# yanqinJiang/Animate3D

Measured on AMD Instinct MI355X. Metric: UNet denoise-steps/sec, 4view×16frame×512² MV-VDM @1/2/4/8 GPU, higher is better.
Workload: dtype bf16; 1 GPU; BASELINE config 2: 4 views x 16 frames x 512^2 px (64x64 latent), CFG-doubled batch V=8 videos, one MVUNetMotionModel.forward per step, SD1.5 MV-VDM UNet 1.53 B params, seeded synthetic weights; parallelism=single GPU

## Files before the change

animate3d_amd/csrc/temporal_attn.hip:

```cpp
#include "common.h"


namespace {

constexpr int SLAB = 320;
constexpr int SL = 40;
constexpr int NSL = SLAB / SL;

struct TAParams {
  const uint16_t* Q; const uint16_t* K; const uint16_t* V; int64_t ld;
  int64_t ldq;
  uint16_t* O; int64_t ldo;
  int videos, frames; int64_t L; int heads; float scale_log2;
  int64_t npix;
  int q_f0, q_frames, kv_fpr; int64_t kv_rs;
};

typedef short s16x4_t __attribute__((ext_vector_type(4)));
typedef _Float16 f16x4_t __attribute__((ext_vector_type(4)));
A3D_DEV f32x4_t mfma16k16(const u32x2_t& a, const u32x2_t& b, const f32x4_t& c) {
#ifdef A3D_STORAGE_F16
  return __builtin_amdgcn_mfma_f32_16x16x16f16(__builtin_bit_cast(f16x4_t, a), __builtin_bit_cast(f16x4_t, b), c, 0, 0, 0);
#else
  return __builtin_amdgcn_mfma_f32_16x16x16bf16_1k(__builtin_bit_cast(s16x4_t, a), __builtin_bit_cast(s16x4_t, b), c, 0, 0, 0);
#endif
}

template <int FP, int D>
__global__ __launch_bounds__(NSL * FP) void temporal_attn_mfma_kernel(const TAParams p) {
  constexpr int ROWB = SLAB + 8;
  constexpr int FB = FP / 16;
  constexpr int KS = (D + 15) / 16;
  constexpr int NH = SLAB / D;
  constexpr int NT = NSL * FP, NW = NT / 64;
  extern __shared__ __attribute__((aligned(16))) uint16_t smem[];
  const int F = p.frames;
  const int tid = threadIdx.x, lane = tid & 63, wid = tid >> 6;
  const int64_t pix = blockIdx.x < p.npix ? (int64_t)blockIdx.x : p.npix - 1;
  const int c0 = blockIdx.y * SLAB;
  const int64_t v = pix / p.L, l = pix % p.L;
  constexpr int chunks = SLAB / 8;

  auto src_of = [&](int it) -> const uint16_t* {
    const int ch = it % chunks;
    const int f = (it / chunks) % F;
    const int ten = it / (chunks * F);
    if (ten == 0) {
      int fq = f - p.q_f0;
      if (fq < 0 || fq >= p.q_frames) fq = 0;
      return p.Q + ((v * p.q_frames + fq) * p.L + l) * p.ldq + c0 + ch * 8;
    }
    const int64_t row = (int64_t)(f / p.kv_fpr) * p.kv_rs + (v * p.kv_fpr + f % p.kv_fpr) * p.L + l;
    return (ten == 1 ? p.K : p.V) + row * p.ld + c0 + ch * 8;
  };
  auto dst_of = [&](int it) -> uint16_t* {
// ... 1 lines not shown
    const int f = (it / chunks) % F;
    const int ten = it / (chunks * F);
    return smem + ((size_t)ten * F + f) * ROWB + ch * 8;
  };
  const int items = 3 * F * chunks;
  if (F == FP) {
    constexpr int ITEMS = 3 * FP * chunks, NIT = (ITEMS + NT - 1) / NT;
    u32x4_t stg[NIT];
#pragma unroll
    for (int k = 0; k < NIT; ++k) {
      const int it = tid + k * NT;
      if (ITEMS % NT == 0 || it < ITEMS) stg[k] = *reinterpret_cast<const u32x4_t*>(src_of(it));
    }
#pragma unroll
    for (int k = 0; k < NIT; ++k) {
      const int it = tid + k * NT;
      if (ITEMS % NT == 0 || it < ITEMS) *reinterpret_cast<u32x4_t*>(dst_of(it)) = stg[k];
    }
  } else {
    for (int it = tid; it < items; it += NT) *reinterpret_cast<u32x4_t*>(dst_of(it)) = *reinterpret_cast<const u32x4_t*>(src_of(it));
  }
  __syncthreads();

  const int i16 = lane & 15, k4 = lane >> 4;
  uint16_t* const Qs = smem;
  const uint16_t* const Ks = smem + (size_t)F * ROWB;
  const uint16_t* const Vs = smem + (size_t)2 * F * ROWB;
  for (int h = wid; h < NH; h += NW) {
    const int hc = h * D;
    f32x4_t sT[FB][FB];
    u32x2_t qfr[FB][KS];
#pragma unroll
    for (int ib = 0; ib < FB; ++ib) {
      const int fi = 16 * ib + i16 < F ? 16 * ib + i16 : F - 1;
#pragma unroll
      for (int ks = 0; ks < KS; ++ks) {
        u32x2_t w = *reinterpret_cast<const u32x2_t*>(Qs + (size_t)fi * ROWB + hc + 16 * ks + 4 * k4);
        if (16 * ks + 4 * k4 >= D) w = u32x2_t{0u, 0u};
        qfr[ib][ks] = w;
      }
    }
#pragma unroll
    for (int jb = 0; jb < FB; ++jb) {
      const int fj = 16 * jb + i16 < F ? 16 * jb + i16 : F - 1;
      u32x2_t kfr[KS];
#pragma unroll
      for (int ks = 0; ks < KS; ++ks) {
        kfr[ks] = *reinterpret_cast<const u32x2_t*>(Ks + (size_t)fj * ROWB + hc + 16 * ks + 4 * k4);
        if (16 * ks + 4 * k4 >= D) kfr[ks] = u32x2_t{0u, 0u};
      }
#pragma unroll
      for (int ib = 0; ib < FB; ++ib) {
        f32x4_t acc = {0.f, 0.f, 0.f, 0.f};
#pragma unroll
        for (int ks = 0; ks < KS; ++ks) acc = mfma16k16(kfr[ks], qfr[ib][ks], acc);
        sT[jb][ib] = acc;
      }
    }
    u32x2_t pfr[FB][FB];
    float inv[FB];
#pragma unroll
    for (int ib = 0; ib < FB; ++ib) {
      float mx = -INFINITY;
#pragma unroll
      for (int jb = 0; jb < FB; ++jb)
#pragma unroll
        for (int r = 0; r < 4; ++r) {
          const bool ok = 16 * jb + 4 * k4 + r < F;
          sT[jb][ib][r] = ok ? sT[jb][ib][r] * p.scale_log2 : -INFINITY;
          mx = fmaxf(mx, sT[jb][ib][r]);
        }
      mx = fmaxf(mx, __shfl_xor(mx, 16));
      mx = fmaxf(mx, __shfl_xor(mx, 32));
      float sum = 0.f;
#pragma unroll
      for (int jb = 0; jb < FB; ++jb) {
        float e[4];
#pragma unroll
        for (int r = 0; r < 4; ++r) { e[r] = __builtin_amdgcn_exp2f(sT[jb][ib][r] - mx); sum += e[r]; }
        pfr[jb][ib] = u32x2_t{pack16(e[0], e[1]), pack16(e[2], e[3])};
      }
      sum += __shfl_xor(sum, 16);
      sum += __shfl_xor(sum, 32);
      inv[ib] = 1.f / sum;
    }
#pragma unroll
    for (int db = 0; db < KS; ++db) {
      u32x2_t vfr[FB];
#pragma unroll
      for (int jb = 0; jb < FB; ++jb) {
        const int fj = 16 * jb + 4 * k4 + (i16 >> 2) < F ? 16 * jb + 4 * k4 + (i16 >> 2) : F - 1;
        vfr[jb] = lds_tr16_b64(Vs + (size_t)fj * ROWB + hc + 16 * db + 4 * (i16 & 3));
      }
#pragma unroll
      for (int ib = 0; ib < FB; ++ib) {
        f32x4_t o = {0.f, 0.f, 0.f, 0.f};
#pragma unroll
        for (int jb = 0; jb < FB; ++jb) o = mfma16k16(vfr[jb], pfr[jb][ib], o);
        const int fi = 16 * ib + i16;
        if (16 * db + 4 * k4 < D && fi < F) {
          const u32x2_t w = {pack16(o[0] * inv[ib], o[1] * inv[ib]), pack16(o[2] * inv[ib], o[3] * inv[ib])};
          *reinterpret_cast<u32x2_t*>(Qs + (size_t)fi * ROWB + hc + 16 * db + 4 * k4) = w;
        }
      }
    }
  }
  __syncthreads();
  if ((int64_t)blockIdx.x < p.npix) {
    for (int it = tid; it < p.q_frames * chunks; it += NT) {
      const int ch = it % chunks, fq = it / chunks;
      const u32x4_t w = *reinterpret_cast<const u32x4_t*>(Qs + (size_t)(p.q_f0 + fq) * ROWB + ch * 8);
      *reinterpret_cast<u32x4_t*>(p.O + ((v * p.q_frames + fq) * p.L + l) * p.ldo + c0 + ch * 8) = w;
    }
  }
}

template <int FP, int D>
int launch_mfma(hipStream_t s, const TAParams& p, int C) {
  if (p.npix > 0x7fffffffLL) return A3D_EINVAL;
  const size_t lds = (size_t)3 * p.frames * (SLAB + 8) * sizeof(uint16_t);
  static uint64_t attr_done = 0;
  if (int rc = a3d_once_per_device(attr_done, [] {
        return (int)hipFuncSetAttribute(reinterpret_cast<const void*>(&temporal_attn_mfma_kernel<FP, D>),
                                        hipFuncAttributeMaxDynamicSharedMemorySize, 3 * FP * (SLAB + 8) * 2); })) return rc;
  temporal_attn_mfma_kernel<FP, D><<<dim3((unsigned)p.npix, (unsigned)(C / SLAB)), dim3(NSL * FP), lds, s>>>(p);
  return a3d_launch_status();
}

template <int DP>
// ... 46 lines not shown
```

animate3d_amd/hip_ops.py:

```python
from __future__ import annotations

import ctypes
import os
from dataclasses import dataclass
from typing import Optional

import torch

_LIB_PATH = os.path.join(os.path.dirname(os.path.abspath(__file__)), "lib", "libanimate3d_hip.so")
_lib = None

c_i64, c_int, c_f32, c_vp = ctypes.c_int64, ctypes.c_int, ctypes.c_float, ctypes.c_void_p


class _RowMapC(ctypes.Structure):
    _fields_ = [("gdiv", c_i64), ("ga", c_i64), ("gb", c_i64), ("seg_len", c_i64), ("seg_stride", c_i64), ("ld", c_i64)]


@dataclass(frozen=True)
class RowMap:
    gdiv: int
    ga: int
    gb: int
    seg_len: int
# ... 15 lines not shown
    idx = rowmap_rows(m, groups, step, length, device)
    return bool(int(idx.min()) >= 0 and int(idx.max()) < rows and torch.unique(idx).numel() == rows)


_SIGNATURES = {
    "a3d_version": (ctypes.c_char_p, []),
    "a3d_gemm_bf16": (c_int, [c_vp, c_vp, c_i64, c_vp, c_i64, c_vp, c_vp, c_i64, c_vp, c_i64, c_vp, c_i64, c_i64, c_i64, c_i64, c_f32, c_f32, c_int]),
    "a3d_gemm_ws_bf16": (c_int, [c_vp, c_vp, c_i64, c_vp, c_i64, c_vp, c_vp, c_i64, c_vp, c_i64, c_vp, c_i64, c_i64, c_i64, c_i64, c_f32, c_f32, c_int,
                                 c_vp, c_i64, ctypes.POINTER(c_i64)]),
    "a3d_gemm2_bf16": (c_int, [c_vp, c_vp, c_i64, c_vp, c_i64, c_i64, c_vp, c_i64, c_vp, c_vp, c_i64, c_i64, c_i64, c_i64, c_int]),
    "a3d_gemm_geglu_bf16": (c_int, [c_vp, c_vp, c_i64, c_vp, c_i64, c_vp, c_vp, c_i64, c_i64, c_i64, c_i64, c_int]),
    "a3d_conv3x3_bf16": (c_int, [c_vp, c_vp, c_vp, c_vp, c_vp, c_i64, c_vp, c_vp, c_int, c_int, c_int, c_int, c_int, c_int, c_int, c_int]),
    "a3d_conv3x3_ws_bf16": (c_int, [c_vp, c_vp, c_vp, c_vp, c_vp, c_i64, c_vp, c_vp, c_int, c_int, c_int, c_int, c_int, c_int, c_int, c_int,
                                    c_vp, c_i64, ctypes.POINTER(c_i64)]),
    "a3d_flash_attn_bf16": (c_int, [c_vp, c_vp, c_vp, c_vp, c_vp, ctypes.POINTER(_RowMapC), ctypes.POINTER(_RowMapC), ctypes.POINTER(_RowMapC),
                                    c_int, c_int, c_int, c_i64, c_i64, c_f32, c_f32, c_int]),
    "a3d_flash_attn_counted_bf16": (c_int, [c_vp, c_vp, c_vp, c_vp, c_vp, ctypes.POINTER(_RowMapC), ctypes.POINTER(_RowMapC), ctypes.POINTER(_RowMapC),
                                            c_int, c_int, c_int, c_i64, c_i64, c_f32, c_f32, c_int, c_vp]),
    "a3d_flash_attn2_bf16": (c_int, [c_vp, c_vp, c_vp, c_vp, c_vp, c_vp, c_vp, ctypes.POINTER(_RowMapC), ctypes.POINTER(_RowMapC), ctypes.POINTER(_RowMapC),
                                     ctypes.POINTER(_RowMapC), c_int, c_int, c_int, c_i64, c_i64, c_i64, c_f32, c_f32, c_f32, c_int]),
    "a3d_temporal_attn_bf16": (c_int, [c_vp, c_vp, c_vp, c_vp, c_i64, c_vp, c_i64, c_int, c_int, c_i64, c_int, c_int, c_f32]),
    "a3d_temporal_attn_sharded_bf16": (c_int, [c_vp, c_vp, c_i64, c_vp, c_vp, c_i64, c_vp, c_i64, c_int, c_int, c_i64, c_int, c_int, c_f32,
                                               c_int, c_int, c_int, c_i64]),
    "a3d_group_norm_ws_floats": (c_i64, [c_int, c_i64, c_int]),
    "a3d_group_norm_bf16": (c_int, [c_vp, c_vp, c_vp, c_vp, c_vp, c_vp, c_int, c_i64, c_int, c_int, c_f32, c_int]),
    "a3d_group_norm2_bf16": (c_int, [c_vp, c_vp, c_int, c_vp, c_int, c_vp, c_vp, c_vp, c_vp, c_int, c_i64, c_int, c_f32, c_int]),
    "a3d_group_norm_sums_bf16": (c_int, [c_vp, c_vp, c_vp, c_vp, c_int, c_i64, c_int, c_int]),
    "a3d_group_norm_apply_bf16": (c_int, [c_vp, c_vp, c_vp, c_vp, c_vp, c_vp, c_int, c_i64, c_int, c_int, c_int]),
    "a3d_layer_norm_bf16": (c_int, [c_vp, c_vp, c_vp, c_vp, c_vp, c_vp, c_i64, c_int, c_f32, c_vp, c_i64, c_i64, c_vp, c_i64, c_i64]),
    "a3d_geglu_bf16": (c_int, [c_vp, c_vp, c_i64, c_vp, c_i64, c_i64, c_i64]),
    "a3d_silu_bf16": (c_int, [c_vp, c_vp, c_vp, c_i64]),
    "a3d_activation_bf16": (c_int, [c_vp, c_vp, c_vp, c_i64, c_int]),
    "a3d_concat_bf16": (c_int, [c_vp, c_vp, c_i64, c_vp, c_i64, c_vp, c_i64]),
    "a3d_timestep_embed_bf16": (c_int, [c_vp, c_vp, c_vp, c_int, c_int]),
    "a3d_im2col_in": (c_int, [c_vp, c_vp, c_int, c_vp, c_int, c_int, c_int, c_int, c_int]),
    "a3d_unpack_out": (c_int, [c_vp, c_vp, c_vp, c_int, c_int, c_int, c_int, c_int, c_int]),
    "a3d_gemm_f32out_bf16": (c_int, [c_vp, c_vp, c_i64, c_vp, c_i64, c_vp, c_vp, c_i64, c_i64, c_i64, c_i64, c_f32]),
    "a3d_softmax_rows_f32_bf16": (c_int, [c_vp, c_vp, c_i64, c_vp, c_i64, c_i64, c_i64]),
    "a3d_softmax_rows_bwd_bf16": (c_int, [c_vp, c_vp, c_i64, c_vp, c_i64, c_vp, c_i64, c_i64, c_i64, c_f32]),
    "a3d_im2col_in_bwd": (c_int, [c_vp, c_vp, c_vp, c_int, c_int, c_int, c_int, c_int, c_f32]),
    "a3d_channel_mix_f32": (c_int, [c_vp, c_vp, c_vp, c_vp, c_vp, c_int, c_int, c_int, c_i64, c_f32]),
    "a3d_cfg_ddim_step_f32": (c_int, [c_vp, c_vp, c_vp, c_vp, c_vp, c_i64, c_int, c_int, c_i64, c_f32, c_f32, c_f32]),
    "a3d_flash_attn_bwd_bf16": (c_int, [c_vp, c_vp, c_vp, c_vp, c_vp, c_vp, c_vp, c_vp, c_vp, c_vp,
                                        ctypes.POINTER(_RowMapC), ctypes.POINTER(_RowMapC), ctypes.POINTER(_RowMapC), ctypes.POINTER(_RowMapC),
                                        ctypes.POINTER(_RowMapC), c_int, c_int, c_int, c_i64, c_i64, c_int, c_f32, c_f32, c_int]),
    "a3d_flash_attn_lse_bf16": (c_int, [c_vp, c_vp, c_vp, c_vp, c_vp, ctypes.POINTER(_RowMapC), ctypes.POINTER(_RowMapC), ctypes.POINTER(_RowMapC),
# ... 14 lines not shown
    "a3d_clip_ctrl_f32": (c_int, [c_vp, c_vp, c_f32, c_f32, c_vp]),
    "a3d_adamw_f32": (c_int, [c_vp, c_vp, c_vp, c_vp, c_vp, c_i64, c_f32, c_f32, c_f32, c_f32, c_f32, c_f32, c_f32, c_vp]),
    "a3d_gs_preprocess_f32": (c_int, [c_vp, c_int, c_int, c_vp, c_i64, c_vp, c_i64, c_vp, c_i64, c_vp, c_i64, c_vp, c_i64, c_int, c_int, c_vp, c_i64, c_vp, c_vp, c_vp, c_vp, c_vp, c_int, c_int, c_f32, c_vp, c_vp, c_vp, c_vp, c_vp, c_vp, c_vp]),
    "a3d_gs_duplicate_f32": (c_int, [c_vp, c_int, c_int, c_int, c_int, c_vp, c_vp, c_vp, c_vp, c_vp, c_vp]),
    "a3d_gs_tile_ranges_f32": (c_int, [c_vp, c_vp, c_i64, c_vp, c_i64]),
    "a3d_gs_render_f32": (c_int, [c_vp, c_int, c_int, c_int, c_int, c_vp, c_vp, c_vp, c_vp, c_vp, c_vp, c_vp, c_vp, c_vp, c_vp, c_vp, c_vp, c_vp]),
    "a3d_gs_render_bwd_f32": (c_int, [c_vp, c_int, c_int, c_int, c_int, c_vp, c_vp, c_vp, c_vp, c_vp, c_vp, c_vp, c_vp, c_vp, c_vp, c_vp,
                                      c_vp, c_vp, c_vp]),
    "a3d_gs_preprocess_bwd_f32": (c_int, [c_vp, c_int, c_int, c_vp, c_i64, c_vp, c_i64, c_vp, c_i64, c_vp, c_i64, c_vp, c_i64, c_int, c_int, c_vp, c_i64, c_vp, c_vp, c_vp, c_vp, c_vp, c_int, c_int, c_f32, c_vp, c_vp, c_vp, c_vp, c_vp, c_vp, c_vp, c_vp, c_vp, c_vp, c_vp, c_vp]),
    "a3d_gs_sum_batch_f32": (c_int, [c_vp, c_vp, c_vp, c_int, c_i64]),
}
_UNSUFFIXED_TWINS = ("a3d_im2col_in", "a3d_unpack_out", "a3d_im2col_in_bwd")
for _name in list(_SIGNATURES):
    if _name.endswith("_bf16"):
        _SIGNATURES[_name[:-5] + "_f16"] = _SIGNATURES[_name]
    elif _name in _UNSUFFIXED_TWINS:
        _SIGNATURES[_name + "_f16"] = _SIGNATURES[_name]
EXPORTED_SYMBOLS = tuple(_SIGNATURES)

_DTYPE_CODE = {torch.float32: 0, torch.bfloat16: 1, torch.float16: 2}
A3D_EUNSUPPORTED = -2


def lib_path() -> str:
    return _LIB_PATH


def load_library():
    global _lib
    if _lib is None:
        if not os.path.exists(_LIB_PATH):
            raise RuntimeError(f"{_LIB_PATH} is missing: run `python -m animate3d_amd.build` (or __graft_entry__.build()). "
                               "There is no CPU fallback for the MI355X kernels.")
        lib = ctypes.CDLL(_LIB_PATH)
        for name, (res, args) in _SIGNATURES.items():
            fn = getattr(lib, name)
            fn.restype, fn.argtypes = res, args
        _lib = lib
    return _lib


def _check(rc: int, what: str):
    if rc != 0:
        kind = {-1: "A3D_EINVAL (shape/alignment precondition)", -2: "A3D_EUNSUPPORTED"}.get(rc, f"hipError {rc}")
        raise RuntimeError(f"{what} failed: {kind}")

# ... 205 lines not shown
            assert cnt.dtype == torch.int32 and cnt.is_cuda and cnt.numel() >= 3 and cnt.is_contiguous()
            rc = self.lib.a3d_flash_attn_counted_bf16(self._stream(), _p(q), _p(k), _p(v), _p(o), ctypes.byref(qm), ctypes.byref(km), ctypes.byref(om),
                                                      groups, heads, D, q_len, kv_len, float(D) ** -0.5, out_scale, flags, _p(cnt))
            _check(rc, f"a3d_flash_attn_counted_bf16 groups={groups} heads={heads} D={D} q_len={q_len} kv_len={kv_len}")
            return o
        rc = self.lib.a3d_flash_attn_bf16(self._stream(), _p(q), _p(k), _p(v), _p(o), ctypes.byref(qm), ctypes.byref(km), ctypes.byref(om),
                                          groups, heads, D, q_len, kv_len, float(D) ** -0.5, out_scale, flags)
        _check(rc, f"a3d_flash_attn_bf16 groups={groups} heads={heads} D={D} q_len={q_len} kv_len={kv_len}")
        return o

    def flash_attn2(self, q, k, v, k2, v2, qmap: RowMap, kmap: RowMap, kmap2: RowMap, groups: int, heads: int, q_len: int, kv_len: int,
                    kv_len2: int, *, out_scale2: float = 1.0):
        D = q.shape[1] // heads
        if D not in (40, 80):
            return None
        q, k, v, k2, v2 = self._act(q, "attn.q"), self._act(k, "attn.k"), self._act(v, "attn.v"), self._act(k2, "attn.k2"), self._act(v2, "attn.v2")
        assert k.stride(0) == v.stride(0) and k2.stride(0) == v2.stride(0)
        o = self.empty(q.shape[0], q.shape[1])
        qm, km, km2, om = qmap.c(q.stride(0)), kmap.c(k.stride(0)), kmap2.c(k2.stride(0)), qmap.c(o.stride(0))
        rc = self.lib.a3d_flash_attn2_bf16(self._stream(), _p(q), _p(k), _p(v), _p(k2), _p(v2), _p(o), ctypes.byref(qm), ctypes.byref(km),
                                           ctypes.byref(km2), ctypes.byref(om), groups, heads, D, q_len, kv_len, kv_len2, float(D) ** -0.5,
                                           1.0, out_scale2, 0)
        _check(rc, f"a3d_flash_attn2_bf16 groups={groups} heads={heads} D={D} q_len={q_len} kv_len={kv_len} kv_len2={kv_len2}")
        return o

    def temporal_attn(self, q, k, v, videos: int, frames: int, L: int, heads: int, *, q_f0: int = 0, q_frames: Optional[int] = None,
                      out=None):
        q, k, v = self._act(q, "tattn.q"), self._act(k, "tattn.k"), self._act(v, "tattn.v")
        C = q.shape[1]
        D = C // heads
        assert k.stride(0) == v.stride(0)
        o = self._act(out, "tattn.out") if out is not None else self.empty(q.shape[0], C)
        assert o.shape == (q.shape[0], C)
        if q_frames is None or q_frames == frames:
            assert q.stride(0) == k.stride(0)
            rc = self.lib.a3d_temporal_attn_bf16(self._stream(), _p(q), _p(k), _p(v), q.stride(0), _p(o), o.stride(0),
                                                 videos, frames, L, heads, D, float(D) ** -0.5)
        else:
            assert q.shape[0] == videos * q_frames * L and k.shape[0] == videos * frames * L
            rc = self.lib.a3d_temporal_attn_sharded_bf16(self._stream(), _p(q), q.stride(0), _p(k), _p(v), k.stride(0), _p(o), o.stride(0),
                                                         videos, frames, L, heads, D, float(D) ** -0.5, q_f0, q_frames, q_frames,
                                                         videos * q_frames * L)
        _check(rc, f"a3d_temporal_attn_bf16 videos={videos} frames={frames} L={L} D={D} q_f0={q_f0} q_frames={q_frames}")
        return o

    def group_norm(self, x, B: int, rows: int, gamma, beta, groups: int, eps: float, silu: bool):
# ... 344 lines not shown
```

animate3d_amd/unet.py:

```python
from __future__ import annotations

import math
import os
import re
from types import SimpleNamespace
from typing import Any, Dict, Optional, Tuple, Union

import torch
import torch.nn as nn

from . import modules as M
from .config import UNetConfig
from .embeddings import sine_pos_2d, sinusoidal_pos_1d
from .hip_ops import RowMap, on_model_device


class UNet3DConditionOutput:

    def __init__(self, sample: torch.Tensor):
        self.sample = sample

    def __getitem__(self, i):
        return (self.sample,)[i]


def _rows(w: torch.Tensor, r0: int, r1: Optional[int] = None) -> torch.Tensor:
    r1 = w.shape[0] if r1 is None else r1
    if getattr(w, "_a3d_sink", None) is None:
        return w[r0:r1]
    from .autograd_ops import weight_rows
    return weight_rows(w, r0, r1)


class MVUNetMotionModel(nn.Module):
    def __init__(self, config: Optional[UNetConfig] = None, ops=None, num_views: Optional[int] = None,
                 device: Optional[Union[str, torch.device]] = None, **config_overrides):
        super().__init__()
        cfg = config if config is not None else UNetConfig(**config_overrides)
        self.config = cfg
        self.sample_size = cfg.sample_size
        self.num_views = num_views
        self._ops = ops
        self._ops_auto = False
        self._packed = None
        self._packed_frozen = None
        self._pack_grad = False
        self._train_ops = None
        self._active_ops = None
        self._cond = None
        self.stack_conditioning = True
        self._pe_cache: Dict[Tuple[int, int, int], torch.Tensor] = {}
        self.parallel = None
        self._frames = (0, 0)
        if len(cfg.block_out_channels) != len(cfg.down_has_attn):
            raise ValueError("block_out_channels and down_has_attn must have the same length")
        if 9 * cfg.in_channels > 64:
            raise ValueError(f"in_channels = {cfg.in_channels} is not supported (<= 7; the MV-VDM UNet has 4 — the 9-channel PIA conv_in "
                             "of unet_motion_mv_model.py:312-330 is not on this path)")
        ctx = torch.device(device) if device is not None else torch.device("cpu")
        with ctx:
            self._build(cfg)
            self._install_default_processors()

    def _build(self, cfg: UNetConfig):
        boc = cfg.block_out_channels
        temb_c = boc[0] * 4
        nlev = len(boc)
        self.conv_in = nn.Conv2d(cfg.in_channels, boc[0], 3, padding=1)
        self.time_embedding = M.TimestepEmbedding(boc[0], temb_c)
        if cfg.camera_embedding_dim is not None:
            self.camera_embedding = M.TimestepEmbedding(cfg.camera_embedding_dim, temb_c)
        self.encoder_hid_proj = None
        if cfg.encoder_hid_dim_type == "ip_image_proj":
# ... 355 lines not shown
        tb = m.transformer_blocks[0]
        attns = []
        for a, ln in ((tb.attn1, tb.norm1), (tb.attn2, tb.norm2)):
            pr = a.processor
            if pr.kind != "spatio_temporal":
                raise TypeError("motion-module attention layers need a SpatioTemporalI2VAttnProcessor")
            C = a.to_q.weight.shape[0]
            if hasattr(pr, "time_pos_embed"):
                pe = pr.time_pos_embed.pe[0]
            else:
                pe = sinusoidal_pos_1d(C, self.config.motion_max_seq_length)[0].to(a.to_q.weight.device)
            proc_pe = hasattr(pr, "time_pos_embed")
            ct, cs, ci = pr.blend_coefficients_t() if self._pack_grad else pr.blend_coefficients()
            if self._pack_grad:
                self._coef_tensors.extend(c for c in (ct, cs, ci) if torch.is_tensor(c))
            ns = SimpleNamespace(
                heads=a.heads, spatial=pr.use_spatial_attn, image=pr.use_image_attn,
                spatial_pe=pr.use_spatial_attn and pr.use_spatial_encoding, camera_pe=pr.use_spatial_attn and pr.use_camera_encoding,
                n=(self._f(ln.weight), self._f(ln.bias)),
                qkv=self._wcat([a.to_q.weight, a.to_k.weight, a.to_v.weight]),
                o=(self._w(a.to_out[0].weight), self._f(a.to_out[0].bias)),
                pe_t=self._w(pe), coef=(ct, cs, ci), proc=pr,
                block_pe=not proc_pe)
            if pr.use_spatial_attn:
                ns.qkv_sp = self._wcat([pr.to_k_sp.weight, pr.to_v_sp.weight, pr.to_q_sp.weight])
                ns.osp = (self._w(pr.to_out_sp.weight), self._f(pr.to_out_sp.bias))
            if pr.use_image_attn:
                ns.qkv_img = self._wcat([pr.to_k_i2v.weight, pr.to_v_i2v.weight, pr.to_q_i2v.weight])
                ns.oimg = (self._w(pr.to_out_i2v.weight), self._f(pr.to_out_i2v.bias))
            ns.om = None
            if not self._pack_grad and (pr.use_spatial_attn or pr.use_image_attn):
                parts = [(ct, a.to_out[0])]
                if pr.use_spatial_attn:
                    parts.append((cs, pr.to_out_sp))
                if pr.use_image_attn:
                    parts.append((ci, pr.to_out_i2v))
                bias = None
                for c, lin in parts:
                    if lin.bias is not None:
                        bias = float(c) * lin.bias.detach().float() if bias is None else bias + float(c) * lin.bias.detach().float()
                ns.om = (self._w(torch.cat([float(c) * lin.weight.detach().float() for c, lin in parts], dim=1)), self._f(bias))
            attns.append(ns)
        out = SimpleNamespace(norm=(self._f(m.norm.weight), self._f(m.norm.bias)),
                              pin=(self._w(m.proj_in.weight), self._f(m.proj_in.bias)),
                              attns=attns,
                              pout=(self._w(m.proj_out.weight), self._f(m.proj_out.bias)))
# ... 252 lines not shown
            cat = ops.empty(n1.shape[0], 2 * C)
            self._mv_attention(n1, pk.qkv, C, V, n, F, L, pk.heads, i2v=True, out_a=cat[:, :C], out_ai=cat[:, C:])
            return ops.gemm(cat, pk.o1m[0], pk.o1m[1], residual=residual)
        a, ai, _ = self._mv_attention(n1, pk.qkv, C, V, n, F, L, pk.heads, i2v=pk.i2v)
        if pk.i2v:
            a = ops.gemm(ai, pk.oi2v[0], pk.oi2v[1], residual=a)
        return ops.gemm(a, pk.o1[0], pk.o1[1], residual=residual)

    def _motion_attn(self, h, nt, ns, nimg, a, V, n, F, L):
        ops = self.ops
        C = nt.shape[1]
        ct, cs, ci = a.coef

        par = self.parallel if (self.parallel is not None and self.parallel.world > 1) else None
        fsh = par is not None and par.frame_shards > 1
        F_all, f0 = self._frames
        merged = a.om is not None and self._active_ops is None
        nblk = 1 + int(a.spatial) + int(a.image)
        cat = ops.empty(nt.shape[0], nblk * C) if merged else None
        blk = lambda i: {} if cat is None else {"out": cat[:, i * C:(i + 1) * C]}

        def temporal_branch(nt=nt, a=a):
            if not fsh:
                qkv = ops.gemm(nt, a.qkv)
                return ops.temporal_attn(qkv[:, :C], qkv[:, C:2 * C], qkv[:, 2 * C:], V, F, L, a.heads, **blk(0))
            kv = ops.gemm(nt, _rows(a.qkv, C))
            pending = par.all_gather_frames_start(kv)
            q = ops.gemm(nt, _rows(a.qkv, 0, C))
            kv_all = par.all_gather_frames_finish(pending)
            return ops.temporal_attn(q, kv_all[:, :C], kv_all[:, C:], V, F_all, L, a.heads, q_f0=f0, q_frames=F, **blk(0))
        if a.spatial:
            asp, _, at = self._mv_attention(ns, a.qkv_sp, C, V, n, F, L, a.heads, i2v=False, overlap=temporal_branch,
                                            out_a=None if cat is None else cat[:, C:2 * C])
        else:
            at = temporal_branch()
        if not merged:
            out = ops.gemm(at, a.o[0], a.o[1], residual=h, alpha=ct, beta=1.0)
            if a.spatial:
                out = ops.gemm(asp, a.osp[0], a.osp[1], residual=out, alpha=cs, beta=1.0)
        if a.image:
            qm = RowMap(gdiv=1, ga=L, gb=0, seg_len=L, seg_stride=0)
            if fsh:
                x0 = nimg.view(V, F, L, C)[:, 0].reshape(V * L, C) if par.frame_rank == 0 else None
                kv0 = ops.gemm(par.broadcast_frame0(x0, (V * L, C), nimg.dtype, nimg.device), _rows(a.qkv_img, 0, 2 * C))
                qi = ops.gemm(nimg, _rows(a.qkv_img, 2 * C))
                ai = ops.flash_attn(qi, kv0[:, :C], kv0[:, C:], qm, RowMap(gdiv=F, ga=L, gb=0, seg_len=L, seg_stride=0), V * F, a.heads, L, L,
# ... 363 lines not shown
```

include/animate3d_hip.h:

```cpp
#ifndef ANIMATE3D_HIP_H
#define ANIMATE3D_HIP_H

#include <stdint.h>

#ifdef __cplusplus
extern "C" {
#endif

typedef void* a3d_stream_t;

enum {
  A3D_OK = 0,
  A3D_EINVAL = -1,
  A3D_EUNSUPPORTED = -2
};

enum { A3D_F32 = 0, A3D_BF16 = 1, A3D_F16 = 2 };

const char* a3d_version(void);

typedef struct a3d_rowmap {
  int64_t gdiv, ga, gb;
  int64_t seg_len, seg_stride;
  int64_t ld;
// ... 33 lines not shown

#define A3D_ATTN_ACCUMULATE 1
#define A3D_ATTN_CAUSAL 2
#define A3D_ATTN_EXACT 4
#define A3D_ATTN_PLAIN 8
int a3d_flash_attn_bf16(a3d_stream_t stream, const void* Q, const void* K, const void* V, void* O,
                        const a3d_rowmap* qmap, const a3d_rowmap* kmap, const a3d_rowmap* omap,
                        int groups, int heads, int head_dim, int64_t q_len, int64_t kv_len,
                        float scale, float out_scale, int accumulate);

int a3d_flash_attn_counted_bf16(a3d_stream_t stream, const void* Q, const void* K, const void* V, void* O,
                                const a3d_rowmap* qmap, const a3d_rowmap* kmap, const a3d_rowmap* omap,
                                int groups, int heads, int head_dim, int64_t q_len, int64_t kv_len,
                                float scale, float out_scale, int accumulate, unsigned int* counters);

int a3d_flash_attn2_bf16(a3d_stream_t stream, const void* Q, const void* K, const void* V, const void* K2, const void* V2, void* O,
                         const a3d_rowmap* qmap, const a3d_rowmap* kmap, const a3d_rowmap* kmap2, const a3d_rowmap* omap,
                         int groups, int heads, int head_dim, int64_t q_len, int64_t kv_len, int64_t kv_len2,
                         float scale, float out_scale, float out_scale2, int accumulate);

int a3d_temporal_attn_bf16(a3d_stream_t stream, const void* Q, const void* K, const void* V, int64_t ldqkv,
                           void* O, int64_t ldo, int videos, int frames, int64_t L, int heads,
                           int head_dim, float scale);

int a3d_temporal_attn_sharded_bf16(a3d_stream_t stream, const void* Q, int64_t ldq, const void* K, const void* V, int64_t ldkv,
                                   void* O, int64_t ldo, int videos, int frames, int64_t L, int heads,
                                   int head_dim, float scale, int q_f0, int q_frames, int kv_frames_per_block,
                                   int64_t kv_block_stride);

int64_t a3d_group_norm_ws_floats(int B, int64_t rows, int groups);
int a3d_group_norm_bf16(a3d_stream_t stream, const void* X, void* Y, const float* gamma, const float* beta,
                        float* ws, int B, int64_t rows, int C, int groups, float eps, int silu);

int a3d_group_norm2_bf16(a3d_stream_t stream, const void* Xa, int Ca, const void* Xb, int Cb, void* Y, const float* gamma,
                         const float* beta, float* ws, int B, int64_t rows, int groups, float eps, int silu);

int a3d_group_norm_sums_bf16(a3d_stream_t stream, const void* X, float* ws, double* sums, int B, int64_t rows, int C, int groups);
int a3d_group_norm_apply_bf16(a3d_stream_t stream, const void* X, void* Y, const float* gamma, const float* beta,
                              const float* stats, int B, int64_t rows, int C, int groups, int silu);

int a3d_layer_norm_bf16(a3d_stream_t stream, const void* X, void* Y1, void* Y2, const float* gamma,
                        const float* beta, int64_t M, int C, float eps,
                        const void* pe1, int64_t pe1_div, int64_t pe1_mod,
                        const void* pe2, int64_t pe2_div, int64_t pe2_mod);

int a3d_geglu_bf16(a3d_stream_t stream, const void* X, int64_t ldx, void* Y, int64_t ldy, int64_t M, int64_t N);
// ... 113 lines not shown
                        const float* bias, void* Y, int64_t ldy, int64_t M, int64_t N2, int64_t K, int flags);
int a3d_conv3x3_f16(a3d_stream_t stream, const void* X, const void* Wp, const float* bias,
                     const void* rowbias, int64_t rb_div, const void* R, void* Y,
                     int B, int H, int W, int Cin, int Cout, int stride, int up2x, int flags);
int a3d_conv3x3_ws_f16(a3d_stream_t stream, const void* X, const void* Wp, const float* bias,
                       const void* rowbias, int64_t rb_div, const void* R, void* Y,
                       int B, int H, int W, int Cin, int Cout, int stride, int up2x, int flags,
                       void* ws, int64_t ws_bytes, int64_t* ws_needed);
int a3d_flash_attn_f16(a3d_stream_t stream, const void* Q, const void* K, const void* V, void* O,
                        const a3d_rowmap* qmap, const a3d_rowmap* kmap, const a3d_rowmap* omap,
                        int groups, int heads, int head_dim, int64_t q_len, int64_t kv_len,
                        float scale, float out_scale, int accumulate);
int a3d_flash_attn_counted_f16(a3d_stream_t stream, const void* Q, const void* K, const void* V, void* O,
                               const a3d_rowmap* qmap, const a3d_rowmap* kmap, const a3d_rowmap* omap,
                               int groups, int heads, int head_dim, int64_t q_len, int64_t kv_len,
                               float scale, float out_scale, int accumulate, unsigned int* counters);
int a3d_flash_attn2_f16(a3d_stream_t stream, const void* Q, const void* K, const void* V, const void* K2, const void* V2, void* O,
                        const a3d_rowmap* qmap, const a3d_rowmap* kmap, const a3d_rowmap* kmap2, const a3d_rowmap* omap,
                        int groups, int heads, int head_dim, int64_t q_len, int64_t kv_len, int64_t kv_len2,
                        float scale, float out_scale, float out_scale2, int accumulate);
int a3d_temporal_attn_f16(a3d_stream_t stream, const void* Q, const void* K, const void* V, int64_t ldqkv,
                           void* O, int64_t ldo, int videos, int frames, int64_t L, int heads,
                           int head_dim, float scale);
int a3d_temporal_attn_sharded_f16(a3d_stream_t stream, const void* Q, int64_t ldq, const void* K, const void* V, int64_t ldkv,
                                   void* O, int64_t ldo, int videos, int frames, int64_t L, int heads,
                                   int head_dim, float scale, int q_f0, int q_frames, int kv_frames_per_block,
                                   int64_t kv_block_stride);
int a3d_group_norm_f16(a3d_stream_t stream, const void* X, void* Y, const float* gamma, const float* beta,
                        float* ws, int B, int64_t rows, int C, int groups, float eps, int silu);
int a3d_group_norm2_f16(a3d_stream_t stream, const void* Xa, int Ca, const void* Xb, int Cb, void* Y, const float* gamma,
                        const float* beta, float* ws, int B, int64_t rows, int groups, float eps, int silu);
int a3d_group_norm_sums_f16(a3d_stream_t stream, const void* X, float* ws, double* sums, int B, int64_t rows, int C, int groups);
int a3d_group_norm_apply_f16(a3d_stream_t stream, const void* X, void* Y, const float* gamma, const float* beta,
                              const float* stats, int B, int64_t rows, int C, int groups, int silu);
int a3d_layer_norm_f16(a3d_stream_t stream, const void* X, void* Y1, void* Y2, const float* gamma,
                        const float* beta, int64_t M, int C, float eps,
                        const void* pe1, int64_t pe1_div, int64_t pe1_mod,
                        const void* pe2, int64_t pe2_div, int64_t pe2_mod);
int a3d_geglu_f16(a3d_stream_t stream, const void* X, int64_t ldx, void* Y, int64_t ldy, int64_t M, int64_t N);
int a3d_silu_f16(a3d_stream_t stream, const void* X, void* Y, int64_t n);
int a3d_activation_f16(a3d_stream_t stream, const void* X, void* Y, int64_t n, int mode);
int a3d_concat_f16(a3d_stream_t stream, const void* A, int64_t Ca, const void* Bsrc, int64_t Cb, void* Y, int64_t M);
int a3d_timestep_embed_f16(a3d_stream_t stream, const float* t, void* Y, int V, int dim);
int a3d_im2col_in_f16(a3d_stream_t stream, const void* sample, int dtype, void* Y, int V, int C, int F, int H, int W);
int a3d_unpack_out_f16(a3d_stream_t stream, const void* X, void* Y, int dtype, int V, int C, int F, int H, int W);
int a3d_softmax_rows_f32_f16(a3d_stream_t stream, const float* X, int64_t ldx, void* Y, int64_t ldy, int64_t M, int64_t N);
// ... 39 lines not shown
```

Before: 2.286 denoise-steps/s.

## Fuse temporal QKV projection GEMM with temporal attention in one kernel

```diff
diff --git a/animate3d_amd/csrc/temporal_attn.hip b/animate3d_amd/csrc/temporal_attn.hip
--- a/animate3d_amd/csrc/temporal_attn.hip
+++ b/animate3d_amd/csrc/temporal_attn.hip
@@ -1,4 +1,4 @@
-#include "common.h"
+#include "temporal_attn_core.h"
 
 
 namespace {
@@ -16,21 +16,9 @@
   int q_f0, q_frames, kv_fpr; int64_t kv_rs;
 };
 
-typedef short s16x4_t __attribute__((ext_vector_type(4)));
-typedef _Float16 f16x4_t __attribute__((ext_vector_type(4)));
-A3D_DEV f32x4_t mfma16k16(const u32x2_t& a, const u32x2_t& b, const f32x4_t& c) {
-#ifdef A3D_STORAGE_F16
-  return __builtin_amdgcn_mfma_f32_16x16x16f16(__builtin_bit_cast(f16x4_t, a), __builtin_bit_cast(f16x4_t, b), c, 0, 0, 0);
-#else
-  return __builtin_amdgcn_mfma_f32_16x16x16bf16_1k(__builtin_bit_cast(s16x4_t, a), __builtin_bit_cast(s16x4_t, b), c, 0, 0, 0);
-#endif
-}
-
 template <int FP, int D>
 __global__ __launch_bounds__(NSL * FP) void temporal_attn_mfma_kernel(const TAParams p) {
   constexpr int ROWB = SLAB + 8;
-  constexpr int FB = FP / 16;
-  constexpr int KS = (D + 15) / 16;
   constexpr int NH = SLAB / D;
   constexpr int NT = NSL * FP, NW = NT / 64;
   extern __shared__ __attribute__((aligned(16))) uint16_t smem[];
@@ -78,89 +66,10 @@
   }
   __syncthreads();
 
-  const int i16 = lane & 15, k4 = lane >> 4;
   uint16_t* const Qs = smem;
   const uint16_t* const Ks = smem + (size_t)F * ROWB;
   const uint16_t* const Vs = smem + (size_t)2 * F * ROWB;
-  for (int h = wid; h < NH; h += NW) {
-    const int hc = h * D;
-    f32x4_t sT[FB][FB];
-    u32x2_t qfr[FB][KS];
-#pragma unroll
-    for (int ib = 0; ib < FB; ++ib) {
-      const int fi = 16 * ib + i16 < F ? 16 * ib + i16 : F - 1;
-#pragma unroll
-      for (int ks = 0; ks < KS; ++ks) {
-        u32x2_t w = *reinterpret_cast<const u32x2_t*>(Qs + (size_t)fi * ROWB + hc + 16 * ks + 4 * k4);
-        if (16 * ks + 4 * k4 >= D) w = u32x2_t{0u, 0u};
-        qfr[ib][ks] = w;
-      }
-    }
-#pragma unroll
-    for (int jb = 0; jb < FB; ++jb) {
-      const int fj = 16 * jb + i16 < F ? 16 * jb + i16 : F - 1;
-      u32x2_t kfr[KS];
-#pragma unroll
-      for (int ks = 0; ks < KS; ++ks) {
-        kfr[ks] = *reinterpret_cast<const u32x2_t*>(Ks + (size_t)fj * ROWB + hc + 16 * ks + 4 * k4);
-        if (16 * ks + 4 * k4 >= D) kfr[ks] = u32x2_t{0u, 0u};
-      }
-#pragma unroll
-      for (int ib = 0; ib < FB; ++ib) {
-        f32x4_t acc = {0.f, 0.f, 0.f, 0.f};
-#pragma unroll
-        for (int ks = 0; ks < KS; ++ks) acc = mfma16k16(kfr[ks], qfr[ib][ks], acc);
-        sT[jb][ib] = acc;
-      }
-    }
-    u32x2_t pfr[FB][FB];
-    float inv[FB];
-#pragma unroll
-    for (int ib = 0; ib < FB; ++ib) {
-      float mx = -INFINITY;
-#pragma unroll
-      for (int jb = 0; jb < FB; ++jb)
-#pragma unroll
-        for (int r = 0; r < 4; ++r) {
-          const bool ok = 16 * jb + 4 * k4 + r < F;
-          sT[jb][ib][r] = ok ? sT[jb][ib][r] * p.scale_log2 : -INFINITY;
-          mx = fmaxf(mx, sT[jb][ib][r]);
-        }
-      mx = fmaxf(mx, __shfl_xor(mx, 16));
-      mx = fmaxf(mx, __shfl_xor(mx, 32));
-      float sum = 0.f;
-#pragma unroll
-      for (int jb = 0; jb < FB; ++jb) {
-        float e[4];
-#pragma unroll
-        for (int r = 0; r < 4; ++r) { e[r] = __builtin_amdgcn_exp2f(sT[jb][ib][r] - mx); sum += e[r]; }
-        pfr[jb][ib] = u32x2_t{pack16(e[0], e[1]), pack16(e[2], e[3])};
-      }
-      sum += __shfl_xor(sum, 16);
-      sum += __shfl_xor(sum, 32);
-      inv[ib] = 1.f / sum;
-    }
-#pragma unroll
-    for (int db = 0; db < KS; ++db) {
-      u32x2_t vfr[FB];
-#pragma unroll
-      for (int jb = 0; jb < FB; ++jb) {
-        const int fj = 16 * jb + 4 * k4 + (i16 >> 2) < F ? 16 * jb + 4 * k4 + (i16 >> 2) : F - 1;
-        vfr[jb] = lds_tr16_b64(Vs + (size_t)fj * ROWB + hc + 16 * db + 4 * (i16 & 3));
-      }
-#pragma unroll
-      for (int ib = 0; ib < FB; ++ib) {
-        f32x4_t o = {0.f, 0.f, 0.f, 0.f};
-#pragma unroll
-        for (int jb = 0; jb < FB; ++jb) o = mfma16k16(vfr[jb], pfr[jb][ib], o);
-        const int fi = 16 * ib + i16;
-        if (16 * db + 4 * k4 < D && fi < F) {
-          const u32x2_t w = {pack16(o[0] * inv[ib], o[1] * inv[ib]), pack16(o[2] * inv[ib], o[3] * inv[ib])};
-          *reinterpret_cast<u32x2_t*>(Qs + (size_t)fi * ROWB + hc + 16 * db + 4 * k4) = w;
-        }
-      }
-    }
-  }
+  for (int h = wid; h < NH; h += NW) temporal_attn_head<FP, D>(Qs + h * D, Ks + h * D, Vs + h * D, ROWB, F, p.scale_log2, lane);
   __syncthreads();
   if ((int64_t)blockIdx.x < p.npix) {
     for (int it = tid; it < p.q_frames * chunks; it += NT) {
diff --git a/animate3d_amd/csrc/temporal_attn_core.h b/animate3d_amd/csrc/temporal_attn_core.h
--- /dev/null
+++ b/animate3d_amd/csrc/temporal_attn_core.h
@@ -0,0 +1,97 @@
+#pragma once
+#include "common.h"
+
+typedef short s16x4_t __attribute__((ext_vector_type(4)));
+typedef _Float16 f16x4_t __attribute__((ext_vector_type(4)));
+A3D_DEV f32x4_t mfma16k16(const u32x2_t& a, const u32x2_t& b, const f32x4_t& c) {
+#ifdef A3D_STORAGE_F16
+  return __builtin_amdgcn_mfma_f32_16x16x16f16(__builtin_bit_cast(f16x4_t, a), __builtin_bit_cast(f16x4_t, b), c, 0, 0, 0);
+#else
+  return __builtin_amdgcn_mfma_f32_16x16x16bf16_1k(__builtin_bit_cast(s16x4_t, a), __builtin_bit_cast(s16x4_t, b), c, 0, 0, 0);
+#endif
+}
+
+template <int FP, int D>
+A3D_DEV void temporal_attn_head(uint16_t* const Qh, const uint16_t* const Kh, const uint16_t* const Vh, const int rs, const int F,
+                                const float scale_log2, const int lane) {
+#pragma clang fp contract(off)
+  constexpr int FB = FP / 16;
+  constexpr int KS = (D + 15) / 16;
+  const int i16 = lane & 15, k4 = lane >> 4;
+  f32x4_t sT[FB][FB];
+  u32x2_t qfr[FB][KS];
+#pragma unroll
+  for (int ib = 0; ib < FB; ++ib) {
+    const int fi = 16 * ib + i16 < F ? 16 * ib + i16 : F - 1;
+#pragma unroll
+    for (int ks = 0; ks < KS; ++ks) {
+      u32x2_t w = *reinterpret_cast<const u32x2_t*>(Qh + (size_t)fi * rs + 16 * ks + 4 * k4);
+      if (16 * ks + 4 * k4 >= D) w = u32x2_t{0u, 0u};
+      qfr[ib][ks] = w;
+    }
+  }
+#pragma unroll
+  for (int jb = 0; jb < FB; ++jb) {
+    const int fj = 16 * jb + i16 < F ? 16 * jb + i16 : F - 1;
+    u32x2_t kfr[KS];
+#pragma unroll
+    for (int ks = 0; ks < KS; ++ks) {
+      kfr[ks] = *reinterpret_cast<const u32x2_t*>(Kh + (size_t)fj * rs + 16 * ks + 4 * k4);
+      if (16 * ks + 4 * k4 >= D) kfr[ks] = u32x2_t{0u, 0u};
+    }
+#pragma unroll
+    for (int ib = 0; ib < FB; ++ib) {
+      f32x4_t acc = {0.f, 0.f, 0.f, 0.f};
+#pragma unroll
+      for (int ks = 0; ks < KS; ++ks) acc = mfma16k16(kfr[ks], qfr[ib][ks], acc);
+      sT[jb][ib] = acc;
+    }
+  }
+  u32x2_t pfr[FB][FB];
+  float inv[FB];
+#pragma unroll
+  for (int ib = 0; ib < FB; ++ib) {
+    float mx = -INFINITY;
+#pragma unroll
+    for (int jb = 0; jb < FB; ++jb)
+#pragma unroll
+      for (int r = 0; r < 4; ++r) {
+        const bool ok = 16 * jb + 4 * k4 + r < F;
+        sT[jb][ib][r] = ok ? sT[jb][ib][r] * scale_log2 : -INFINITY;
+        mx = fmaxf(mx, sT[jb][ib][r]);
+      }
+    mx = fmaxf(mx, __shfl_xor(mx, 16));
+    mx = fmaxf(mx, __shfl_xor(mx, 32));
+    float sum = 0.f;
+#pragma unroll
+    for (int jb = 0; jb < FB; ++jb) {
+      float e[4];
+#pragma unroll
+      for (int r = 0; r < 4; ++r) { e[r] = __builtin_amdgcn_exp2f(sT[jb][ib][r] - mx); sum += e[r]; }
+      pfr[jb][ib] = u32x2_t{pack16(e[0], e[1]), pack16(e[2], e[3])};
+    }
+    sum += __shfl_xor(sum, 16);
+    sum += __shfl_xor(sum, 32);
+    inv[ib] = 1.f / sum;
+  }
+#pragma unroll
+  for (int db = 0; db < KS; ++db) {
+    u32x2_t vfr[FB];
+#pragma unroll
+    for (int jb = 0; jb < FB; ++jb) {
+      const int fj = 16 * jb + 4 * k4 + (i16 >> 2) < F ? 16 * jb + 4 * k4 + (i16 >> 2) : F - 1;
+      vfr[jb] = lds_tr16_b64(Vh + (size_t)fj * rs + 16 * db + 4 * (i16 & 3));
+    }
+#pragma unroll
+    for (int ib = 0; ib < FB; ++ib) {
+      f32x4_t o = {0.f, 0.f, 0.f, 0.f};
+#pragma unroll
+      for (int jb = 0; jb < FB; ++jb) o = mfma16k16(vfr[jb], pfr[jb][ib], o);
+      const int fi = 16 * ib + i16;
+      if (16 * db + 4 * k4 < D && fi < F) {
+        const u32x2_t w = {pack16(o[0] * inv[ib], o[1] * inv[ib]), pack16(o[2] * inv[ib], o[3] * inv[ib])};
+        *reinterpret_cast<u32x2_t*>(Qh + (size_t)fi * rs + 16 * db + 4 * k4) = w;
+      }
+    }
+  }
+}
diff --git a/animate3d_amd/csrc/temporal_qkv_attn.hip b/animate3d_amd/csrc/temporal_qkv_attn.hip
--- /dev/null
+++ b/animate3d_amd/csrc/temporal_qkv_attn.hip
@@ -0,0 +1,166 @@
+#include "temporal_attn_core.h"
+
+namespace {
+
+constexpr int TBM = 128;
+constexpr int NT = 256;
+constexpr int TBN = 256;
+constexpr int CG = 80;
+constexpr int QKV = 3 * CG;
+constexpr int IRS = QKV + 8;
+constexpr int STAGE = (TBM + TBN) * 128;
+constexpr int SMEM = STAGE > TBM * IRS * 2 ? STAGE : TBM * IRS * 2;
+
+struct TQParams {
+  const uint16_t* X; int64_t ldx;
+  const uint16_t* W; int64_t K;
+  uint16_t* O; int64_t ldo;
+  int64_t L;
+  int64_t tiles;
+  int groups;
+  float scale_log2;
+};
+
+template <int FP, int D>
+__global__ __launch_bounds__(NT, 2) void temporal_qkv_attn_kernel(const TQParams p) {
+  constexpr int NPIX = TBM / FP;
+  constexpr int HG = CG / D;
+  extern __shared__ __attribute__((aligned(16))) uint16_t smem[];
+  char* const smem_b = reinterpret_cast<char*>(smem);
+  const int tid = threadIdx.x, lane = tid & 63, wid = tid >> 6;
+  const int wm = wid >> 1, wn = wid & 1;
+  const int l31 = lane & 31, g = lane >> 5;
+
+  const int64_t t = xcd_remap(blockIdx.x, gridDim.x);
+  const int grp = (int)(t % p.groups);
+  const int64_t tile_m = t / p.groups;
+  const int64_t pgs = p.L / NPIX;
+  const int64_t v = tile_m / pgs, l0 = (tile_m % pgs) * NPIX;
+  auto grow = [&](int r) -> int64_t { return (v * FP + r / NPIX) * p.L + l0 + r % NPIX; };
+
+  constexpr int XI = TBM / 32, WI = TBN / 32;
+  const int ch = tid & 7, r0 = tid >> 3;
+  const uint32_t sdst = (uint32_t)(r0 * 128 + ((ch ^ ((r0 >> 1) & 7)) << 4));
+  const uint16_t* xsrc[XI];
+#pragma unroll
+  for (int i = 0; i < XI; ++i) xsrc[i] = p.X + grow(r0 + 32 * i) * p.ldx + ch * 8;
+  const uint16_t* const wsrc = p.W + ((int64_t)grp * TBN + r0) * p.K + ch * 8;
+  u32x4_t rx[XI], rw[WI];
+  auto gload = [&](int kt) __attribute__((always_inline)) {
+#pragma unroll
+    for (int i = 0; i < XI; ++i) rx[i] = *reinterpret_cast<const u32x4_t*>(xsrc[i] + kt * 64);
+#pragma unroll
+    for (int i = 0; i < WI; ++i) rw[i] = *reinterpret_cast<const u32x4_t*>(wsrc + (int64_t)32 * i * p.K + kt * 64);
+  };
+  auto lstore = [&]() __attribute__((always_inline)) {
+#pragma unroll
+    for (int i = 0; i < XI; ++i) *reinterpret_cast<u32x4_t*>(smem_b + sdst + 32 * 128 * i) = rx[i];
+#pragma unroll
+    for (int i = 0; i < WI; ++i) *reinterpret_cast<u32x4_t*>(smem_b + TBM * 128 + sdst + 32 * 128 * i) = rw[i];
+  };
+
+  f32x16_t acc[4][2];
+#pragma unroll
+  for (int a = 0; a < 4; ++a)
+#pragma unroll
+    for (int b = 0; b < 2; ++b)
+#pragma unroll
+      for (int r = 0; r < 16; ++r) acc[a][b][r] = 0.f;
+
+  const uint32_t koff0 = (uint32_t)((g ^ ((l31 >> 1) & 7)) << 4);
+  const uint32_t xrd = (uint32_t)(wm * 64 + l31) * 128u;
+  const uint32_t wrd = (uint32_t)(TBM * 128) + (uint32_t)(wn * 128 + l31) * 128u;
+  const int nk = (int)(p.K / 64);
+  gload(0);
+  for (int kt = 0; kt < nk; ++kt) {
+    lstore();
+    __syncthreads();
+    if (kt + 1 < nk) gload(kt + 1);
+    const char* const xs = smem_b + xrd;
+    const char* const ws = smem_b + wrd;
+#pragma unroll
+    for (int ks = 0; ks < 4; ++ks) {
+      const uint32_t ko = koff0 ^ (uint32_t)(ks << 5);
+      u32x4_t fx[2], fw[4];
+#pragma unroll
+      for (int tm = 0; tm < 2; ++tm) fx[tm] = *reinterpret_cast<const u32x4_t*>(xs + tm * 4096 + ko);
+#pragma unroll
+      for (int tn = 0; tn < 4; ++tn) fw[tn] = *reinterpret_cast<const u32x4_t*>(ws + tn * 4096 + ko);
+#pragma unroll
+      for (int tn = 0; tn < 4; ++tn)
+#pragma unroll
+        for (int tm = 0; tm < 2; ++tm) acc[tn][tm] = mfma32(fw[tn], fx[tm], acc[tn][tm]);
+    }
+    __syncthreads();
+  }
+
+  uint16_t* const img = smem;
+#pragma unroll
+  for (int tn = 0; tn < 4; ++tn)
+#pragma unroll
+    for (int tm = 0; tm < 2; ++tm)
+#pragma unroll
+      for (int q = 0; q < 4; ++q) {
+        const int col = wn * 128 + tn * 32 + 8 * q + 4 * g;
+        const int row = wm * 64 + tm * 32 + l31;
+        if (col < QKV) {
+          const u32x2_t w = {pack16(acc[tn][tm][4 * q], acc[tn][tm][4 * q + 1]), pack16(acc[tn][tm][4 * q + 2], acc[tn][tm][4 * q + 3])};
+          *reinterpret_cast<u32x2_t*>(img + row * IRS + col) = w;
+        }
+      }
+  __syncthreads();
+
+#pragma unroll
+  for (int j = 0; j < NPIX * HG / (NT / 64); ++j) {
+    const int idx = wid + (NT / 64) * j;
+    const int pl = idx % NPIX, h = idx / NPIX;
+    uint16_t* const qh = img + pl * IRS + h * D;
+    temporal_attn_head<FP, D>(qh, qh + CG, qh + 2 * CG, NPIX * IRS, FP, p.scale_log2, lane);
+  }
+  __syncthreads();
+
+  constexpr int OCH = CG / 8;
+#pragma unroll
+  for (int k = 0; k < TBM * OCH / NT; ++k) {
+    const int it = tid + NT * k;
+    const int row = it / OCH, c = it % OCH;
+    const u32x4_t w = *reinterpret_cast<const u32x4_t*>(img + row * IRS + c * 8);
+    *reinterpret_cast<u32x4_t*>(p.O + grow(row) * p.ldo + grp * CG + c * 8) = w;
+  }
+}
+
+template <int FP, int D>
+int launch(hipStream_t s, const TQParams& p) {
+  static uint64_t attr_done = 0;
+  if (int rc = a3d_once_per_device(attr_done, [] {
+        return (int)hipFuncSetAttribute(reinterpret_cast<const void*>(&temporal_qkv_attn_kernel<FP, D>),
+                                        hipFuncAttributeMaxDynamicSharedMemorySize, SMEM); })) return rc;
+  temporal_qkv_attn_kernel<FP, D><<<dim3((unsigned)p.tiles), dim3(NT), SMEM, s>>>(p);
+  return a3d_launch_status();
+}
+
+}
+
+extern "C" int A3D_FN(a3d_temporal_qkv_attn)(a3d_stream_t stream, const void* X, int64_t ldx, const void* Wp, int64_t K,
+                                           void* O, int64_t ldo, int videos, int frames, int64_t L, int heads,
+                                           int head_dim, float scale) {
+  if (!X || !Wp || !O || videos <= 0 || L <= 0 || heads <= 0) return A3D_EINVAL;
+  if (frames != 16 && frames != 32) return A3D_EINVAL;
+  if (head_dim != 40 && head_dim != 80) return A3D_EINVAL;
+  const int64_t C = (int64_t)heads * head_dim;
+  if (C % CG != 0) return A3D_EINVAL;
+  if (K < 64 || K % 64 != 0 || ldx < K || ldx % 8 != 0 || ldo < C || ldo % 8 != 0) return A3D_EINVAL;
+  if ((reinterpret_cast<uintptr_t>(X) | reinterpret_cast<uintptr_t>(Wp) | reinterpret_cast<uintptr_t>(O)) & 15u) return A3D_EINVAL;
+  const int npix = TBM / frames;
+  if (L % npix != 0) return A3D_EINVAL;
+  TQParams p{};
+  p.X = (const uint16_t*)X; p.ldx = ldx; p.W = (const uint16_t*)Wp; p.K = K;
+  p.O = (uint16_t*)O; p.ldo = ldo; p.L = L;
+  p.groups = (int)(C / CG);
+  p.tiles = (int64_t)videos * (L / npix) * p.groups;
+  if (p.tiles > 0x7fffffffLL) return A3D_EINVAL;
+  p.scale_log2 = scale * 1.4426950408889634f;
+  hipStream_t s = (hipStream_t)stream;
+  if (frames == 16) return head_dim == 40 ? launch<16, 40>(s, p) : launch<16, 80>(s, p);
+  return head_dim == 40 ? launch<32, 40>(s, p) : launch<32, 80>(s, p);
+}
diff --git a/animate3d_amd/hip_ops.py b/animate3d_amd/hip_ops.py
--- a/animate3d_amd/hip_ops.py
+++ b/animate3d_amd/hip_ops.py
@@ -61,6 +61,7 @@
     "a3d_temporal_attn_bf16": (c_int, [c_vp, c_vp, c_vp, c_vp, c_i64, c_vp, c_i64, c_int, c_int, c_i64, c_int, c_int, c_f32]),
     "a3d_temporal_attn_sharded_bf16": (c_int, [c_vp, c_vp, c_i64, c_vp, c_vp, c_i64, c_vp, c_i64, c_int, c_int, c_i64, c_int, c_int, c_f32,
                                                c_int, c_int, c_int, c_i64]),
+    "a3d_temporal_qkv_attn_bf16": (c_int, [c_vp, c_vp, c_i64, c_vp, c_i64, c_vp, c_i64, c_int, c_int, c_i64, c_int, c_int, c_f32]),
     "a3d_group_norm_ws_floats": (c_i64, [c_int, c_i64, c_int]),
     "a3d_group_norm_bf16": (c_int, [c_vp, c_vp, c_vp, c_vp, c_vp, c_vp, c_int, c_i64, c_int, c_int, c_f32, c_int]),
     "a3d_group_norm2_bf16": (c_int, [c_vp, c_vp, c_int, c_vp, c_int, c_vp, c_vp, c_vp, c_vp, c_int, c_i64, c_int, c_f32, c_int]),
@@ -121,6 +122,25 @@
 A3D_EUNSUPPORTED = -2
 
 
+TQKV_GROUP = 80
+TQKV_ROWS = 256
+
+
+def pack_temporal_qkv_weight(qkv: torch.Tensor) -> torch.Tensor:
+    C, K = qkv.shape[0] // 3, qkv.shape[1]
+    if qkv.shape[0] != 3 * C or C % TQKV_GROUP:
+        raise ValueError(f"pack_temporal_qkv_weight: [3C, K] with C a multiple of {TQKV_GROUP} expected, got {tuple(qkv.shape)}")
+    G = C // TQKV_GROUP
+    w = qkv.new_zeros(G, TQKV_ROWS, K)
+    w[:, :3 * TQKV_GROUP] = qkv.reshape(3, G, TQKV_GROUP, K).transpose(0, 1).reshape(G, 3 * TQKV_GROUP, K)
+    return w.reshape(G * TQKV_ROWS, K)
+
+
+def unpack_temporal_qkv_weight(wp: torch.Tensor) -> torch.Tensor:
+    G, K = wp.shape[0] // TQKV_ROWS, wp.shape[1]
+    return wp.reshape(G, TQKV_ROWS, K)[:, :3 * TQKV_GROUP].reshape(G, 3, TQKV_GROUP, K).transpose(0, 1).reshape(3 * G * TQKV_GROUP, K)
+
+
 def lib_path() -> str:
     return _LIB_PATH
 
@@ -372,6 +392,20 @@
                                            ctypes.byref(km2), ctypes.byref(om), groups, heads, D, q_len, kv_len, kv_len2, float(D) ** -0.5,
                                            1.0, out_scale2, 0)
         _check(rc, f"a3d_flash_attn2_bf16 groups={groups} heads={heads} D={D} q_len={q_len} kv_len={kv_len} kv_len2={kv_len2}")
+        return o
+
+    def temporal_qkv_attn(self, x, wp, videos: int, frames: int, L: int, heads: int, *, out=None):
+        x, wp = self._act(x, "tqkv.x"), self._act(wp, "tqkv.w")
+        M, K = x.shape
+        assert wp.shape[1] == K and wp.is_contiguous() and wp.shape[0] % TQKV_ROWS == 0, (x.shape, wp.shape)
+        C = wp.shape[0] // TQKV_ROWS * TQKV_GROUP
+        D = C // heads
+        assert M == videos * frames * L and D * heads == C, (M, videos, frames, L, C, heads)
+        o = self._act(out, "tqkv.out") if out is not None else self.empty(M, C)
+        assert o.shape == (M, C)
+        rc = self.lib.a3d_temporal_qkv_attn_bf16(self._stream(), _p(x), x.stride(0), _p(wp), K, _p(o), o.stride(0),
+                                                 videos, frames, L, heads, D, float(D) ** -0.5)
+        _check(rc, f"a3d_temporal_qkv_attn_bf16 videos={videos} frames={frames} L={L} C={C} D={D} K={K}")
         return o
 
     def temporal_attn(self, q, k, v, videos: int, frames: int, L: int, heads: int, *, q_f0: int = 0, q_frames: Optional[int] = None,
diff --git a/animate3d_amd/unet.py b/animate3d_amd/unet.py
--- a/animate3d_amd/unet.py
+++ b/animate3d_amd/unet.py
@@ -12,7 +12,7 @@
 from . import modules as M
 from .config import UNetConfig
 from .embeddings import sine_pos_2d, sinusoidal_pos_1d
-from .hip_ops import RowMap, on_model_device
+from .hip_ops import RowMap, on_model_device, pack_temporal_qkv_weight
 
 
 class UNet3DConditionOutput:
@@ -49,6 +49,7 @@
         self._active_ops = None
         self._cond = None
         self.stack_conditioning = True
+        self.fuse_temporal_qkv = True
         self._pe_cache: Dict[Tuple[int, int, int], torch.Tensor] = {}
         self.parallel = None
         self._frames = (0, 0)
@@ -450,6 +451,7 @@
                 o=(self._w(a.to_out[0].weight), self._f(a.to_out[0].bias)),
                 pe_t=self._w(pe), coef=(ct, cs, ci), proc=pr,
                 block_pe=not proc_pe)
+            ns.qkv_t = pack_temporal_qkv_weight(ns.qkv) if (not self._pack_grad and C in (320, 640) and C // a.heads in (40, 80)) else None
             if pr.use_spatial_attn:
                 ns.qkv_sp = self._wcat([pr.to_k_sp.weight, pr.to_v_sp.weight, pr.to_q_sp.weight])
                 ns.osp = (self._w(pr.to_out_sp.weight), self._f(pr.to_out_sp.bias))
@@ -748,6 +750,9 @@
 
         def temporal_branch(nt=nt, a=a):
             if not fsh:
+                if (self._active_ops is None and self.fuse_temporal_qkv and getattr(a, "qkv_t", None) is not None and F in (16, 32)
+                        and L % (128 // F) == 0 and hasattr(ops, "temporal_qkv_attn")):
+                    return ops.temporal_qkv_attn(nt, a.qkv_t, V, F, L, a.heads, **blk(0))
                 qkv = ops.gemm(nt, a.qkv)
                 return ops.temporal_attn(qkv[:, :C], qkv[:, C:2 * C], qkv[:, 2 * C:], V, F, L, a.heads, **blk(0))
             kv = ops.gemm(nt, _rows(a.qkv, C))
diff --git a/include/animate3d_hip.h b/include/animate3d_hip.h
--- a/include/animate3d_hip.h
+++ b/include/animate3d_hip.h
@@ -79,6 +79,10 @@
 int a3d_temporal_attn_bf16(a3d_stream_t stream, const void* Q, const void* K, const void* V, int64_t ldqkv,
                            void* O, int64_t ldo, int videos, int frames, int64_t L, int heads,
                            int head_dim, float scale);
+
+int a3d_temporal_qkv_attn_bf16(a3d_stream_t stream, const void* X, int64_t ldx, const void* Wp, int64_t K,
+                               void* O, int64_t ldo, int videos, int frames, int64_t L, int heads,
+                               int head_dim, float scale);
 
 int a3d_temporal_attn_sharded_bf16(a3d_stream_t stream, const void* Q, int64_t ldq, const void* K, const void* V, int64_t ldkv,
                                    void* O, int64_t ldo, int videos, int frames, int64_t L, int heads,
@@ -238,6 +242,9 @@
 int a3d_temporal_attn_f16(a3d_stream_t stream, const void* Q, const void* K, const void* V, int64_t ldqkv,
                            void* O, int64_t ldo, int videos, int frames, int64_t L, int heads,
                            int head_dim, float scale);
+int a3d_temporal_qkv_attn_f16(a3d_stream_t stream, const void* X, int64_t ldx, const void* Wp, int64_t K,
+                               void* O, int64_t ldo, int videos, int frames, int64_t L, int heads,
+                               int head_dim, float scale);
 int a3d_temporal_attn_sharded_f16(a3d_stream_t stream, const void* Q, int64_t ldq, const void* K, const void* V, int64_t ldkv,
                                    void* O, int64_t ldo, int videos, int frames, int64_t L, int heads,
                                    int head_dim, float scale, int q_f0, int q_frames, int kv_frames_per_block,
```

Result: no change. 2.277 denoise-steps/s (median of 2 runs) (-0.4%).
